# CV-Project2025/Project-NeRF

Measured on AMD Instinct MI355X. Metric: train rays/sec + 800x800 render FPS, NeRF-Synthetic Lego; PSNR parity, higher is better.
Workload: dtype bf16; 1 GPU; Part 2 vanilla NeRF train step (L10/L4 Fourier, 8x256 skip-4 MLP, view 128), batch sampling included; rays_per_gpu=4096, samples_per_ray=64, global_rays=4096, parallelism=ray-dp1, weights=random init (seed 0), frames=100 x 800x800 RGBA resident in HBM (uniform noise)

## Files before the change

include/nerf_hip.h:

```cpp
#ifndef NERF_HIP_H
#define NERF_HIP_H

#include <stddef.h>
#include <stdint.h>

#ifdef __cplusplus
extern "C" {
#endif

#define NERF_OK 0
#define NERF_EINVAL (-22)
#define NERF_ELAUNCH (-5)
#define NERF_ENOSYS (-38)

#define NERF_ABI_VERSION 11

typedef void* nerf_stream_t;

const char* nerf_last_error(void);
int nerf_abi_version(void);

int nerf_set_option(const char* name, int value);
int nerf_get_option(const char* name, int* value_out);

int nerf_sample_rays(const float* rays_o, const float* rays_d, const float* u,
                     int64_t n_rays, int n_samples, float near_plane, float far_plane,
                     float* z_out, float* pts_out, float* dirs_out, nerf_stream_t stream);

int nerf_gather_rays(const float* images, const float* poses, const int64_t* img_idx, const int64_t* pix_y,
                     const int64_t* pix_x, int64_t batch, int n_images, int H, int W, float focal,
                     float scene_scale, float* rays_o, float* rays_d, float* rgba, nerf_stream_t stream);

int nerf_gather_batch(const float* images, const float* poses, const int64_t* flat_idx, int64_t batch, int n_images,
                      int H, int W, float focal, float scene_scale, const float* bg, float* rays_o, float* rays_d,
                      float* rgba, float* target, nerf_stream_t stream);

int nerf_train_batch(const float* images, const float* poses, int n_images, int H, int W, float focal,
                     float scene_scale, const float* bg, uint64_t seed, uint64_t counter, int64_t batch,
                     int n_samples, float near_plane, float far_plane, int perturb, float* rays_o, float* rays_d,
                     float* rgba, float* target, float* z_out, nerf_stream_t stream);

int nerf_train_batch_shard(const float* images, const float* poses, int n_images, int H, int W, float focal,
                     float scene_scale, const float* bg, uint64_t seed, uint64_t counter, int64_t first_ray, int64_t batch,
                     int n_samples, float near_plane, float far_plane, int perturb, float* rays_o, float* rays_d,
                     float* rgba, float* target, float* z_out, nerf_stream_t stream);

int nerf_active_mask(const float* pts, int64_t n, const uint8_t* binary_grid, int resolution,
                     float bound, uint8_t* mask_out, int64_t* idx_out, nerf_stream_t stream);

int nerf_sample_compact(const float* rays_o, const float* rays_d, const float* u, int64_t n_rays,
                        int n_samples, float near_plane, float far_plane, const uint8_t* binary_grid,
                        int resolution, float bound, float* z_out, int* slot_of_sample, float* pts_compact,
                        float* dirs_compact, unsigned* active_count, nerf_stream_t stream);
int nerf_sample_compact_jitter(const float* rays_o, const float* rays_d, uint64_t seed, uint64_t counter,
                               int64_t n_rays, int n_samples, float near_plane, float far_plane,
                               const uint8_t* binary_grid, int resolution, float bound, float* z_out,
                               int* slot_of_sample, float* pts_compact, float* dirs_compact,
                               unsigned* active_count, nerf_stream_t stream);
int nerf_sample_compact_jitter_shard(const float* rays_o, const float* rays_d, uint64_t seed, uint64_t counter,
                                     int64_t first_ray, int64_t n_rays, int n_samples, float near_plane, float far_plane,
                                     const uint8_t* binary_grid, int resolution, float bound, float* z_out,
                                     int* slot_of_sample, float* pts_compact, float* dirs_compact,
                                     unsigned* active_count, nerf_stream_t stream);
#define NERF_COMPACT_CHAIN_WORDS 40
int nerf_sample_compact_jitter_chain(const float* rays_o, const float* rays_d, uint64_t seed, uint64_t counter,
                                     int64_t first_ray, int64_t n_rays, int n_samples, float near_plane, float far_plane,
                                     const uint8_t* binary_grid, int resolution, float bound, float* z_out,
                                     int* slot_of_sample, float* pts_compact, float* dirs_compact,
                                     unsigned* chain_state, int turn, unsigned* count_host, unsigned seq, nerf_stream_t stream);

int nerf_train_batch_compact(const float* images, const float* poses, int n_images, int H, int W, float focal,
                             float scene_scale, const float* bg, uint64_t seed, uint64_t counter, int64_t first_ray,
                             int64_t batch, int n_samples, float near_plane, float far_plane,
                             const uint8_t* binary_grid, int resolution, float bound, float* rays_o, float* rays_d,
                             float* rgba, float* target, float* z_out, int* slot_of_sample, float* pts_compact,
                             float* dirs_compact, unsigned* active_count, nerf_stream_t stream);
int nerf_train_batch_compact_chain(const float* images, const float* poses, int n_images, int H, int W, float focal,
                                   float scene_scale, const float* bg, uint64_t seed, uint64_t counter, int64_t first_ray,
                                   int64_t batch, int n_samples, float near_plane, float far_plane,
                                   const uint8_t* binary_grid, int resolution, float bound, float* rays_o, float* rays_d,
                                   float* rgba, float* target, float* z_out, int* slot_of_sample, float* pts_compact,
                                   float* dirs_compact, unsigned* chain_state, int turn, unsigned* count_host, unsigned seq,
                                   nerf_stream_t stream);

size_t nerf_sample_compact_ordered_scratch_bytes(int64_t n_rays, int n_samples);
int nerf_sample_compact_ordered(const float* rays_o, const float* rays_d, const float* u, int draw, uint64_t seed, uint64_t counter,
                                int64_t first_ray, int64_t n_rays, int n_samples, float near_plane, float far_plane,
                                const uint8_t* binary_grid, int resolution, float bound, float* z_out, int* slot_of_sample,
                                float* pts_compact, float* dirs_compact, unsigned* active_count, void* scratch,
                                size_t scratch_bytes, nerf_stream_t stream);

int nerf_sample_pdf(const float* z_coarse, const float* weights, const float* u, int64_t n_rays,
                    int n_coarse, int n_fine, float* z_out, nerf_stream_t stream);

int nerf_grid_lattice(float bound, int resolution, float* pts_out, nerf_stream_t stream);
int nerf_grid_update(const float* sigma, float* grid, uint8_t* binary_grid, int64_t n_cells,
                     float decay, int dynamic, float threshold, unsigned long long* active_count,
                     nerf_stream_t stream);

int nerf_fourier_encode(const float* x, int64_t n, int dim, int n_freq, float* out,
                        nerf_stream_t stream);

int nerf_composite_fwd(const float* rgb, const float* sigma, const float* z, const float* rays_d,
                       const float* bg, int64_t bg_rows, const float* extra,
                       int64_t n_rays, int n_samples,
                       float* out_rgb, float* out_depth, float* out_acc,
                       float* extra_map, float* weights_out, nerf_stream_t stream);

int nerf_composite_bwd(const float* rgb, const float* sigma, const float* z, const float* rays_d,
                       const float* bg, int64_t bg_rows, const float* extra,
                       const float* g_rgb, const float* g_depth, const float* g_acc,
                       const float* g_extra, int64_t n_rays, int n_samples,
                       float* d_rgb, float* d_sigma, float* d_extra, nerf_stream_t stream);

int nerf_composite_fwd_indexed(const float* rgb_compact, const float* sigma_compact, const int* slot_of_sample,
                               const float* z, const float* rays_d, const float* bg, int64_t bg_rows,
                               int64_t n_rays, int n_samples, float* out_rgb, float* out_depth,
                               float* out_acc, nerf_stream_t stream);
int nerf_composite_bwd_indexed(const float* rgb_compact, const float* sigma_compact, const int* slot_of_sample,
                               const float* z, const float* rays_d, const float* bg, int64_t bg_rows,
                               const float* g_rgb, const float* g_depth, const float* g_acc, int64_t n_rays,
                               int n_samples, float* d_rgb_compact, float* d_sigma_compact,
                               nerf_stream_t stream);

#define NERF_MLP_PARAM_COUNT 595844

size_t nerf_mlp_packed_bytes(void);
int nerf_mlp_pack(const float* params_f32, void* packed, nerf_stream_t stream);
int nerf_mlp_pack_streams(const float* params_f32, void* packed, int which, nerf_stream_t stream);

size_t nerf_mlp_stash_bytes(int64_t n);
int nerf_mlp_fwd(const void* packed, const float* rays_o, const float* rays_d, const float* z,
                 int64_t n, int n_samples, float* rgb, float* sigma, void* stash,
                 nerf_stream_t stream);

int nerf_mlp_fwd_encoded(const void* packed, const float* x_enc, const float* d_enc, int64_t n, float* rgb,
                         float* sigma, void* stash, nerf_stream_t stream);

size_t nerf_mlp_bwd_workspace_bytes(int64_t n);
int nerf_mlp_bwd(const void* packed, const void* stash, const float* rgb, const float* sigma,
                 const float* d_rgb, const float* d_sigma, int64_t n, float* grads_f32,
                 void* workspace, nerf_stream_t stream);
int nerf_mlp_bwd_dgrad(const void* packed, const void* stash, const float* rgb, const float* sigma,
                       const float* d_rgb, const float* d_sigma, int64_t n, void* workspace,
                       nerf_stream_t stream);
int nerf_mlp_bwd_dgrad_ex(const void* packed, const void* stash, const float* rgb, const float* sigma,
// ... 254 lines not shown
```

project-nerf_amd/_lib.py:

```python
import ctypes
import os

_HERE = os.path.dirname(os.path.abspath(__file__))
LIB_PATH = os.path.join(_HERE, "libnerf_hip.so")

c_f32p = ctypes.c_void_p
c_ptr = ctypes.c_void_p
i64 = ctypes.c_int64
i32 = ctypes.c_int
f32 = ctypes.c_float
size_t = ctypes.c_size_t

PROTOTYPES = {
    "nerf_last_error": (ctypes.c_char_p, []),
    "nerf_abi_version": (i32, []),
    "nerf_set_option": (i32, [ctypes.c_char_p, i32]),
    "nerf_get_option": (i32, [ctypes.c_char_p, ctypes.POINTER(i32)]),
    "nerf_sample_rays": (i32, [c_ptr, c_ptr, c_ptr, i64, i32, f32, f32, c_ptr, c_ptr, c_ptr, c_ptr]),
    "nerf_gather_rays": (i32, [c_ptr, c_ptr, c_ptr, c_ptr, c_ptr, i64, i32, i32, i32, f32, f32, c_ptr, c_ptr, c_ptr, c_ptr]),
    "nerf_gather_batch": (i32, [c_ptr, c_ptr, c_ptr, i64, i32, i32, i32, f32, f32, c_ptr, c_ptr, c_ptr, c_ptr, c_ptr, c_ptr]),
    "nerf_train_batch": (i32, [c_ptr, c_ptr, i32, i32, i32, f32, f32, c_ptr, ctypes.c_uint64, ctypes.c_uint64, i64, i32, f32, f32,
                               i32, c_ptr, c_ptr, c_ptr, c_ptr, c_ptr, c_ptr]),
    "nerf_train_batch_shard": (i32, [c_ptr, c_ptr, i32, i32, i32, f32, f32, c_ptr, ctypes.c_uint64, ctypes.c_uint64, i64, i64, i32, f32, f32,
                                     i32, c_ptr, c_ptr, c_ptr, c_ptr, c_ptr, c_ptr]),
    "nerf_active_mask": (i32, [c_ptr, i64, c_ptr, i32, f32, c_ptr, c_ptr, c_ptr]),
    "nerf_sample_compact": (i32, [c_ptr, c_ptr, c_ptr, i64, i32, f32, f32, c_ptr, i32, f32, c_ptr, c_ptr, c_ptr, c_ptr, c_ptr, c_ptr]),
    "nerf_sample_compact_jitter": (i32, [c_ptr, c_ptr, ctypes.c_uint64, ctypes.c_uint64, i64, i32, f32, f32, c_ptr, i32, f32,
                                         c_ptr, c_ptr, c_ptr, c_ptr, c_ptr, c_ptr]),
    "nerf_sample_compact_jitter_shard": (i32, [c_ptr, c_ptr, ctypes.c_uint64, ctypes.c_uint64, i64, i64, i32, f32, f32, c_ptr, i32, f32,
                                               c_ptr, c_ptr, c_ptr, c_ptr, c_ptr, c_ptr]),
    "nerf_sample_compact_jitter_chain": (i32, [c_ptr, c_ptr, ctypes.c_uint64, ctypes.c_uint64, i64, i64, i32, f32, f32, c_ptr, i32, f32,
                                               c_ptr, c_ptr, c_ptr, c_ptr, c_ptr, i32, c_ptr, ctypes.c_uint32, c_ptr]),
    "nerf_train_batch_compact": (i32, [c_ptr, c_ptr, i32, i32, i32, f32, f32, c_ptr, ctypes.c_uint64, ctypes.c_uint64, i64, i64, i32, f32, f32,
                                       c_ptr, i32, f32, c_ptr, c_ptr, c_ptr, c_ptr, c_ptr, c_ptr, c_ptr, c_ptr, c_ptr, c_ptr]),
    "nerf_train_batch_compact_chain": (i32, [c_ptr, c_ptr, i32, i32, i32, f32, f32, c_ptr, ctypes.c_uint64, ctypes.c_uint64, i64, i64, i32, f32,
                                             f32, c_ptr, i32, f32, c_ptr, c_ptr, c_ptr, c_ptr, c_ptr, c_ptr, c_ptr, c_ptr, c_ptr, i32, c_ptr,
                                             ctypes.c_uint32, c_ptr]),
    "nerf_composite_fwd_indexed": (i32, [c_ptr, c_ptr, c_ptr, c_ptr, c_ptr, c_ptr, i64, i64, i32, c_ptr, c_ptr, c_ptr, c_ptr]),
    "nerf_composite_bwd_indexed": (i32, [c_ptr, c_ptr, c_ptr, c_ptr, c_ptr, c_ptr, i64, c_ptr, c_ptr, c_ptr, i64, i32, c_ptr, c_ptr, c_ptr]),
    "nerf_sample_pdf": (i32, [c_ptr, c_ptr, c_ptr, i64, i32, i32, c_ptr, c_ptr]),
    "nerf_grid_lattice": (i32, [f32, i32, c_ptr, c_ptr]),
    "nerf_grid_update": (i32, [c_ptr, c_ptr, c_ptr, i64, f32, i32, f32, c_ptr, c_ptr]),
    "nerf_fourier_encode": (i32, [c_ptr, i64, i32, i32, c_ptr, c_ptr]),
    "nerf_composite_fwd": (i32, [c_ptr, c_ptr, c_ptr, c_ptr, c_ptr, i64, c_ptr, i64, i32,
                                 c_ptr, c_ptr, c_ptr, c_ptr, c_ptr, c_ptr]),
    "nerf_composite_bwd": (i32, [c_ptr, c_ptr, c_ptr, c_ptr, c_ptr, i64, c_ptr, c_ptr, c_ptr, c_ptr,
                                 c_ptr, i64, i32, c_ptr, c_ptr, c_ptr, c_ptr]),
    "nerf_render_rays_workspace_bytes": (size_t, [i64, i32]),
    "nerf_render_rays_fwd": (i32, [c_ptr, c_ptr, c_ptr, i64, i32, f32, f32, c_ptr, i64, i64, c_ptr, c_ptr, c_ptr, c_ptr, c_ptr]),
    "nerf_instant_render_workspace_bytes": (size_t, [i64, i32]),
    "nerf_instant_render_rays_fwd": (i32, [c_ptr, c_ptr, c_ptr, i32, c_ptr, c_ptr, c_ptr, c_ptr, c_ptr, f32, c_ptr, i32, f32, c_ptr, c_ptr, i64, i32,
                                           f32, f32, c_ptr, i64, i64, c_ptr, c_ptr, c_ptr, c_ptr, c_ptr]),
    "nerf_render_rays_grid_workspace_bytes": (size_t, [i64, i32]),
    "nerf_render_rays_grid_fwd": (i32, [c_ptr, c_ptr, i32, f32, c_ptr, c_ptr, i64, i32, f32, f32, c_ptr, i64, i64, c_ptr, c_ptr, c_ptr, c_ptr,
                                        c_ptr]),
    "nerf_mlp_packed_bytes": (size_t, []),
    "nerf_mlp_pack": (i32, [c_ptr, c_ptr, c_ptr]),
    "nerf_mlp_pack_streams": (i32, [c_ptr, c_ptr, i32, c_ptr]),
    "nerf_mlp_stash_bytes": (size_t, [i64]),
    "nerf_mlp_fwd": (i32, [c_ptr, c_ptr, c_ptr, c_ptr, i64, i32, c_ptr, c_ptr, c_ptr, c_ptr]),
    "nerf_mlp_fwd_encoded": (i32, [c_ptr, c_ptr, c_ptr, i64, c_ptr, c_ptr, c_ptr, c_ptr]),
    "nerf_mlp_bwd_workspace_bytes": (size_t, [i64]),
    "nerf_mlp_bwd": (i32, [c_ptr, c_ptr, c_ptr, c_ptr, c_ptr, c_ptr, i64, c_ptr, c_ptr, c_ptr]),
    "nerf_mlp_bwd_dgrad": (i32, [c_ptr, c_ptr, c_ptr, c_ptr, c_ptr, c_ptr, i64, c_ptr, c_ptr]),
    "nerf_mlp_bwd_wgrad": (i32, [c_ptr, c_ptr, i64, c_ptr, c_ptr]),
    "nerf_mlp_bwd_dgrad_ex": (i32, [c_ptr, c_ptr, c_ptr, c_ptr, c_ptr, c_ptr, i64, c_ptr, c_ptr, c_ptr]),
    "nerf_composite_mse_bwd": (i32, [c_ptr, c_ptr, c_ptr, c_ptr, c_ptr, c_ptr, i64, c_ptr, f32, i64, i32, c_ptr, c_ptr,
                                     c_ptr, c_ptr, c_ptr, c_ptr, c_ptr]),
    "nerf_mlp_wgrad_part_split": (i64, []),
    "nerf_mlp_bwd_wgrad_part": (i32, [c_ptr, c_ptr, i64, c_ptr, i32, c_ptr]),
    "nerf_hash_encode_fwd": (i32, [c_ptr, i64, c_ptr, i32, c_ptr, c_ptr, c_ptr, c_ptr, c_ptr, f32, c_ptr, c_ptr, c_ptr, c_ptr]),
    "nerf_hash_encode_fwd_f16": (i32, [c_ptr, i64, c_ptr, i32, c_ptr, c_ptr, c_ptr, c_ptr, c_ptr, f32, c_ptr, c_ptr, c_ptr]),
    "nerf_hash_encode_fwd_nat": (i32, [c_ptr, i64, c_ptr, c_ptr, i32, c_ptr, c_ptr, c_ptr, c_ptr, c_ptr, f32, c_ptr, i32, c_ptr]),
    "nerf_hash_encode_fwd_nat_tables": (i32, [c_ptr, i64, c_ptr, i32, i64, i32, c_ptr, c_ptr, c_ptr, c_ptr, c_ptr, f32, c_ptr, i64, i32, c_ptr]),
    "nerf_f32_to_f16": (i32, [c_ptr, c_ptr, i64, c_ptr]),
    "nerf_hash_encode_bwd": (i32, [c_ptr, i64, i32, c_ptr, c_ptr, c_ptr, c_ptr, c_ptr, f32, c_ptr, c_ptr, c_ptr]),
    "nerf_hash_encode_bwd_levels": (i32, [c_ptr, i64, i32, c_ptr, c_ptr, c_ptr, c_ptr, c_ptr, f32, c_ptr, c_ptr, i32, i32, c_ptr]),
    "nerf_hash_encode_bwd_workspace_bytes": (size_t, [i64, i32]),
    "nerf_hash_encode_bwd_ws": (i32, [c_ptr, i64, i32, c_ptr, c_ptr, c_ptr, c_ptr, c_ptr, f32, c_ptr, c_ptr, i32, i32, c_ptr, size_t, c_ptr]),
    "nerf_hash_encode_bwd_ws_store": (i32, [c_ptr, i64, i32, c_ptr, c_ptr, c_ptr, c_ptr, c_ptr, f32, c_ptr, c_ptr, i32, i32, c_ptr, size_t, c_ptr]),
    "nerf_hash_encode_bwd_tables_workspace_bytes": (size_t, [i64, i32, i32]),
    "nerf_hash_encode_bwd_ws_store_tables": (i32, [c_ptr, i64, i32, i64, i32, c_ptr, c_ptr, c_ptr, c_ptr, c_ptr, f32, c_ptr, i64, c_ptr, c_ptr, size_t, c_ptr]),
    "nerf_hash_encode_bwd_ws_store_tables_spec": (i32, [c_ptr, i64, i32, i64, i32, c_ptr, c_ptr, c_ptr, c_ptr, c_ptr, f32, c_ptr, i64, c_ptr, c_ptr, size_t,
                                                        c_ptr, c_ptr]),
    "nerf_hash_encode_fwd_f16_hist": (i32, [c_ptr, i64, c_ptr, i32, c_ptr, c_ptr, c_ptr, c_ptr, c_ptr, f32, c_ptr, c_ptr, size_t, c_ptr]),
    "nerf_hash_encode_bwd_ws_slots": (i32, [c_ptr, i64, i32, ctypes.POINTER(c_ptr), ctypes.POINTER(c_ptr)]),
    "nerf_hash_encode_bwd_ws_store_precounted": (i32, [c_ptr, i64, i32, c_ptr, c_ptr, c_ptr, c_ptr, c_ptr, f32, c_ptr, c_ptr, size_t, c_ptr]),
    "nerf_hash_encode_bwd_spec_begin": (i32, [c_ptr, c_ptr]),
    "nerf_hash_encode_bwd_ws_store_spec": (i32, [c_ptr, i64, i32, c_ptr, c_ptr, c_ptr, c_ptr, c_ptr, f32, c_ptr, c_ptr, c_ptr, size_t, c_ptr, c_ptr]),
    "nerf_imlp_bwd_amax": (i32, [c_ptr, c_ptr, c_ptr, c_ptr, c_ptr, c_ptr, i64, c_ptr, c_ptr, c_ptr, c_ptr]),
    "nerf_hash_encode_bwd_spec_status": (c_ptr, [c_ptr]),
    "nerf_imlp_bwd_lm": (i32, [c_ptr, c_ptr, c_ptr, c_ptr, c_ptr, c_ptr, i64, c_ptr, c_ptr, c_ptr, c_ptr]),
    "nerf_hash_encode_bwd_input": (i32, [c_ptr, i64, c_ptr, i32, c_ptr, c_ptr, c_ptr, c_ptr, c_ptr, f32, c_ptr, c_ptr, c_ptr]),
# ... 21 lines not shown
    "nerf_p4_workspace_bytes": (size_t, [i64]),
    "nerf_p4_infer_workspace_bytes": (size_t, [i64]),
    "nerf_p4_workspace_offset": (size_t, [i64, i32]),
    "nerf_p4_pack": (i32, [c_ptr, c_ptr, c_ptr]),
    "nerf_p4_sample_inputs": (i32, [c_ptr, c_ptr, c_ptr, i64, i32, f32, f32, ctypes.c_uint64, ctypes.c_uint64, i64, c_ptr, c_ptr, c_ptr]),
    "nerf_p4_deform_fwd": (i32, [c_ptr, c_ptr, c_ptr, c_ptr, c_ptr, c_ptr, i64, c_ptr, c_ptr, i32, c_ptr]),
    "nerf_p4_canon_fwd": (i32, [c_ptr, c_ptr, c_ptr, c_ptr, i64, c_ptr, c_ptr, i32, c_ptr]),
    "nerf_p4_canon_bwd": (i32, [c_ptr, c_ptr, c_ptr, c_ptr, c_ptr, c_ptr, i64, c_ptr, c_ptr, c_ptr, c_ptr]),
    "nerf_p4_deform_bwd": (i32, [c_ptr, c_ptr, c_ptr, c_ptr, i64, c_ptr, c_ptr, c_ptr, c_ptr]),
    "nerf_p3_deform_param_count": (i64, []),
    "nerf_p3_deform_packed_bytes": (size_t, []),
    "nerf_p3_deform_workspace_bytes": (size_t, [i64]),
    "nerf_p3_deform_pack": (i32, [c_ptr, c_ptr, c_ptr]),
    "nerf_p3_deform_fwd": (i32, [c_ptr, c_ptr, c_ptr, c_ptr, c_ptr, i64, c_ptr, c_ptr, i32, c_ptr]),
    "nerf_p3_deform_bwd": (i32, [c_ptr, c_ptr, c_ptr, i64, c_ptr, c_ptr]),
    "nerf_p3_canon_param_count": (i64, [i32]),
    "nerf_p3_canon_packed_bytes": (size_t, []),
    "nerf_p3_canon_workspace_bytes": (size_t, [i64]),
    "nerf_p3_canon_pack": (i32, [c_ptr, i32, c_ptr, c_ptr]),
    "nerf_p3_canon_fwd": (i32, [c_ptr, c_ptr, c_ptr, c_ptr, c_ptr, i64, c_ptr, c_ptr, i32, c_ptr]),
    "nerf_p3_canon_bwd": (i32, [c_ptr, c_ptr, c_ptr, c_ptr, c_ptr, c_ptr, c_ptr, i64, i32, c_ptr, c_ptr, c_ptr]),
    "nerf_p1_param_count": (i64, [i32, i32, i32, i32]),
    "nerf_p1_packed_bytes": (size_t, [i32, i32, i32, i32]),
    "nerf_p1_workspace_bytes": (size_t, [i64, i32, i32, i32, i32]),
    "nerf_p1_pack": (i32, [c_ptr, i32, i32, i32, i32, c_ptr, c_ptr]),
    "nerf_p1_fwd": (i32, [c_ptr, c_ptr, i64, i32, i32, i32, i32, c_ptr, c_ptr]),
    "nerf_p1_fwd_loss_bwd": (i32, [c_ptr, c_ptr, c_ptr, c_ptr, c_ptr, i64, i32, i32, i32, i32, c_ptr, c_ptr, c_ptr]),
    "nerf_p2_param_count": (i64, [i32] * 6),
    "nerf_p2_packed_bytes": (size_t, [i32] * 6),
    "nerf_p2_workspace_bytes": (size_t, [i64] + [i32] * 6),
    "nerf_p2_pack": (i32, [c_ptr] + [i32] * 6 + [c_ptr, c_ptr]),
    "nerf_p2_fwd": (i32, [c_ptr, c_ptr, c_ptr, c_ptr, i64, i32] + [i32] * 6 + [c_ptr, c_ptr, c_ptr]),
    "nerf_p2_fwd_train": (i32, [c_ptr, c_ptr, c_ptr, c_ptr, c_ptr, i64, i32] + [i32] * 6 + [c_ptr, c_ptr, c_ptr]),
    "nerf_p2_bwd": (i32, [c_ptr, c_ptr, c_ptr, c_ptr, c_ptr, c_ptr, i64] + [i32] * 6 + [c_ptr, c_ptr]),
    "nerf_imlp_shape_param_count": (i64, [i32] * 3),
    "nerf_imlp_shape_packed_bytes": (size_t, [i32] * 3),
    "nerf_imlp_shape_workspace_bytes": (size_t, [i64] + [i32] * 3),
    "nerf_imlp_shape_hash_operand_offset": (size_t, [i64] + [i32] * 3),
    "nerf_imlp_shape_pack": (i32, [c_ptr] + [i32] * 3 + [c_ptr, c_ptr]),
    "nerf_imlp_shape_fwd": (i32, [c_ptr, c_ptr, c_ptr, i64] + [i32] * 3 + [c_ptr, c_ptr, i32, c_ptr]),
    "nerf_imlp_shape_bwd": (i32, [c_ptr, c_ptr, c_ptr, c_ptr, c_ptr, c_ptr, i64] + [i32] * 3 + [c_ptr, c_ptr, c_ptr]),
    "nerf_tv_codes_bytes": (size_t, [i64]),
    "nerf_tv_normsq_codes": (i32, [c_ptr, c_ptr, i64, i32, f32, f32, c_ptr, i32, c_ptr, c_ptr]),
    "nerf_clip_adamw_small": (i32, [c_ptr, c_ptr, c_ptr, c_ptr, i64, i32, f32, f32, f32, f32, f32, f32, f32, c_ptr, i32, c_ptr]),
    "nerf_adamw_clip_step_tv": (i32, [c_ptr, c_ptr, c_ptr, c_ptr, i64, i32, f32, f32, f32, f32, f32, c_ptr, f32, f32, c_ptr, i64, f32, i64,
                                      f32, i64, i64, f32, c_ptr, c_ptr]),
    "nerf_tv_normsq_codes_piece": (i32, [c_ptr, c_ptr, i64, i64, i32, f32, f32, c_ptr, i32, c_ptr, c_ptr]),
    "nerf_adamw_clip_step_tv_piece": (i32, [c_ptr, c_ptr, c_ptr, c_ptr, i64, i32, f32, f32, f32, f32, f32, c_ptr, f32, f32, c_ptr, f32, i64, i32,
                                            c_ptr, c_ptr]),
    "nerf_adamw_clip_step": (i32, [c_ptr, c_ptr, c_ptr, c_ptr, i64, i32, f32, f32, f32, f32, f32, c_ptr, f32, f32, c_ptr]),
    "nerf_adamw_clip_step_shadow": (i32, [c_ptr, c_ptr, c_ptr, c_ptr, i64, i32, f32, f32, f32, f32, f32, c_ptr, f32, f32, c_ptr, c_ptr]),
}

ABI_VERSION = 11

_lib = None


class NerfHipError(RuntimeError):
    pass


def load():
    global _lib
    if _lib is not None:
        return _lib
    if not os.path.exists(LIB_PATH):
        raise NerfHipError(
            f"{LIB_PATH} not found: build it with `python project-nerf_amd/build.py` "
            "(hipcc --offload-arch=gfx950).  There is no fallback path.")
    import torch
    lib = ctypes.CDLL(LIB_PATH, mode=ctypes.RTLD_GLOBAL)
    for name, (res, args) in PROTOTYPES.items():
        fn = getattr(lib, name)
        fn.restype = res
        fn.argtypes = args
    if lib.nerf_abi_version() != ABI_VERSION:
        raise NerfHipError(f"ABI version mismatch: {LIB_PATH} reports {lib.nerf_abi_version()}, this binding was written against "
                           f"{ABI_VERSION} (rebuild with `python project-nerf_amd/build.py`)")
    _lib = lib
    return lib


NORMSQ_WS_FLOATS = 4136
COMPACT_CHAIN_WORDS = 40
SUM_WS_FLOATS = 12288


def set_option(name: str, value: int) -> None:
    check(load().nerf_set_option(name.encode(), int(value)), f"nerf_set_option({name})")


def get_option(name: str) -> int:
    out = i32(0)
    check(load().nerf_get_option(name.encode(), ctypes.byref(out)), f"nerf_get_option({name})")
    return out.value


def check(code, what):
    if code != 0:
        msg = load().nerf_last_error().decode("utf-8", "replace")
        raise NerfHipError(f"{what} failed ({code}): {msg}")
```

project-nerf_amd/csrc/hierarchical.hip:

```cpp
#include "common.h"

namespace nerf {

constexpr int kMaxCoarse = 256, kMaxTotal = 1024;

__device__ __forceinline__ float wave_inclusive_sum(float v) {
  v += dpp_row_shr<1>(v, 0.0f);
  v += dpp_row_shr<2>(v, 0.0f);
  v += dpp_row_shr<4>(v, 0.0f);
  v += dpp_row_shr<8>(v, 0.0f);
  const int lane = __lane_id();
  const float r0 = lane_read(v, 15), r1 = lane_read(v, 31), r2 = lane_read(v, 47);
  const int row = lane >> 4;
  return v + (row == 0 ? 0.0f : (row == 1 ? r0 : (row == 2 ? r0 + r1 : r0 + r1 + r2)));
}

__global__ void __launch_bounds__(64)
sample_pdf_kernel(const float* __restrict__ z, const float* __restrict__ weights, const float* __restrict__ u,
                  int64_t R, int S, int NF, int P, float* __restrict__ z_out) {
  __shared__ float cdf[kMaxCoarse];
  __shared__ float bins[kMaxCoarse];
  __shared__ float vals[kMaxTotal];
  const int lane = threadIdx.x;
  const int nb = S - 1;
  const int K = (nb + 63) / 64;
  for (int64_t r = blockIdx.x; r < R; r += gridDim.x) {
    const float* zr = z + r * S;
    const float* wr = weights + r * S;
    float local[4], sum = 0.0f;
    for (int k = 0; k < K; ++k) {
      const int i = lane * K + k;
      local[k] = i < S - 2 ? wr[i + 1] + 1e-5f : 0.0f;
      sum += local[k];
    }
    const float incl = wave_inclusive_sum(sum);
    const float total = lane_read(incl, 63);
    float run = incl - sum;
    for (int k = 0; k < K; ++k) {
      const int i = lane * K + k;
      if (i < nb) {
        cdf[i] = run / total;
        bins[i] = 0.5f * (zr[i + 1] + zr[i]);
      }
      run += local[k];
    }
    __syncthreads();
    const float ustep = NF > 1 ? 1.0f / (float)(NF - 1) : 0.0f;
    for (int j = lane; j < NF; j += 64) {
      float uj;
      if (u != nullptr) uj = u[r * NF + j];
      else uj = (j < NF / 2 || NF == 1) ? ustep * (float)j : __builtin_fmaf(-ustep, (float)(NF - 1 - j), 1.0f);
      int lo = 0, hi = nb;
      while (lo < hi) {
        const int mid = (lo + hi) >> 1;
        if (cdf[mid] <= uj) lo = mid + 1; else hi = mid;
      }
      const int below = lo - 1 > 0 ? lo - 1 : 0, above = lo < nb - 1 ? lo : nb - 1;
      float denom = cdf[above] - cdf[below];
      if (denom < 1e-5f) denom = 1.0f;
      const float t = (uj - cdf[below]) / denom;
      vals[S + j] = bins[below] + t * (bins[above] - bins[below]);
    }
    for (int i = lane; i < S; i += 64) vals[i] = zr[i];
    for (int i = S + NF + lane; i < P; i += 64) vals[i] = __builtin_inff();
    __syncthreads();
    for (int k = 2; k <= P; k <<= 1) {
      for (int j = k >> 1; j > 0; j >>= 1) {
        for (int i = lane; i < P; i += 64) {
          const int l = i ^ j;
          if (l > i) {
            const float a = vals[i], b = vals[l];
            const bool up = (i & k) == 0;
            if ((a > b) == up) { vals[i] = b; vals[l] = a; }
          }
        }
        __syncthreads();
      }
    }
    for (int i = lane; i < S + NF; i += 64) z_out[r * (S + NF) + i] = vals[i];
    __syncthreads();
  }
}

}

extern "C" int nerf_sample_pdf(const float* z_coarse, const float* weights, const float* u, int64_t n_rays,
                               int n_coarse, int n_fine, float* z_out, nerf_stream_t stream) {
  using namespace nerf;
  NERF_REQUIRE(n_rays >= 0 && n_coarse >= 3 && n_coarse <= kMaxCoarse && n_fine >= 1 && n_coarse + n_fine <= kMaxTotal,
               "nerf_sample_pdf: n_coarse=%d (3..%d), n_fine=%d, total <= %d", n_coarse, kMaxCoarse, n_fine, kMaxTotal);
  if (n_rays == 0) return NERF_OK;
  NERF_REQUIRE(z_coarse && weights && z_out, "nerf_sample_pdf: NULL pointer");
  int P = 2;
  while (P < n_coarse + n_fine) P <<= 1;
  int64_t blocks = n_rays < 65536 ? n_rays : 65536;
  hipLaunchKernelGGL(sample_pdf_kernel, dim3((int)blocks), dim3(64), 0, as_stream(stream), z_coarse, weights, u, n_rays,
                     n_coarse, n_fine, P, z_out);
  return check_launch("nerf_sample_pdf");
}
```

project-nerf_amd/engine.py:

```python
from __future__ import annotations

import os
from typing import Dict, Optional, Tuple

import torch

from . import flat_params, ops
from .flat_engine import LapSlots, ViewSlots, cosine_lr, render_chunks

Tensor = torch.Tensor


def param_shapes():
    return [(k, shape) for k, _, shape in flat_params.nerf_decoder_table("", 63, 27)]


def default_init(seed: int = 0) -> Tensor:
    g = torch.Generator().manual_seed(seed)
    parts, fan_in = [], 1
    for name, shape in param_shapes():
        if name.endswith("weight"):
            fan_in = shape[1]
        parts.append(((torch.rand(shape, generator=g) * 2 - 1) / fan_in ** 0.5).reshape(-1))
    return torch.cat(parts)
# ... 8 lines not shown


class VanillaNerfEngine:
    def __init__(self, params: Optional[Tensor] = None, device: str = "cuda", lr: float = 5e-4,
                 near: float = 2.0, far: float = 6.0, white_bkgd: bool = True, seed: int = 0,
                 world_size: int = 1, grid_resolution: int = 128, bound: float = 1.5, grid_threshold: float = 0.01):
        self.device = torch.device(device)
        flat = default_init(seed) if params is None else params.detach().float().reshape(-1)
        assert flat.numel() == ops.MLP_PARAM_COUNT
        self.params = flat.to(self.device).contiguous()
        self.exp_avg = torch.zeros_like(self.params)
        self.exp_avg_sq = torch.zeros_like(self.params)
        self.grads = torch.empty_like(self.params)
        self.packed = torch.empty(ops.mlp_packed_bytes(), dtype=torch.uint8, device=self.device)
        self.lr, self.near, self.far = lr, near, far
        self.bg = (torch.ones(3) if white_bkgd else torch.zeros(3)).to(self.device)
        self.step_count = 0
        self.world_size = world_size
        self.grad_scale = torch.full((1,), 1.0 / world_size, device=self.device)
        self._ws: Dict[Tuple[str, int], Tensor] = {}
        self._scalars = torch.zeros(2, 1024, device=self.device)
        self._slots = LapSlots(self._scalars)
        self._infer_stale = False
        self.grid_resolution, self.bound, self.grid_threshold = int(grid_resolution), float(bound), float(grid_threshold)
        self.grid: Optional[Tensor] = None
        self.binary_grid: Optional[Tensor] = None
        self._grid_ws: Dict[Tuple[int, int], Tensor] = {}
        self.seed, self._jitter_counter = int(seed), 0
        self._grid_train_ws: Dict[str, Tensor] = {}
        self.repack()

    def repack(self, training_only: bool = False) -> None:
        ops.mlp_pack(self.params, self.packed, which=1 if training_only else 3)
        self._infer_stale = training_only

    def _inference_weights(self) -> Tensor:
        if self._infer_stale:
            ops.mlp_pack(self.params, self.packed, which=2)
            self._infer_stale = False
        return self.packed

    def state_dict(self, prefix: str = "decoder.") -> Dict[str, Tensor]:
        return {k: v.clone() for k, v in unflatten(self.params, prefix).items()}

    def load_state_dict(self, sd: Dict[str, Tensor], prefix: str = "decoder.") -> None:
        self.params.copy_(flatten_state_dict(sd, prefix).to(self.device))
        self.repack()

    def _buf(self, kind: str, nbytes: int) -> Tensor:
        key = (kind, nbytes)
        if key not in self._ws:
            self._ws[key] = torch.empty(nbytes, dtype=torch.uint8, device=self.device)
        return self._ws[key]

    GRID_SLACK = (1.25, 1 << 20)

    def _grid_buf(self, kind: str, nbytes: int) -> Tensor:
        buf = self._grid_train_ws.get(kind)
        if buf is None or buf.numel() < nbytes:
            buf = None
            self._grid_train_ws.pop(kind, None)
            buf = self._grid_train_ws[kind] = torch.empty(int(nbytes * self.GRID_SLACK[0]) + self.GRID_SLACK[1], dtype=torch.uint8,
                                                          device=self.device)
        return buf

    def prepare_batch(self, rays_o: Tensor, rays_d: Tensor, n_samples: int = 64, u: Optional[Tensor] = None, first_ray: int = 0):
        grid = self._require_grid("prepare_batch")
        jitter = None
        if u is None:
            self._jitter_counter += 1
            jitter = (self.seed, self._jitter_counter)
        return ops.sample_compact_async(rays_o, rays_d, self.near, self.far, n_samples, grid, self.bound, u=u, jitter=jitter,
                                        first_ray=first_ray)

    def _grid_gradients(self, rays_o: Tensor, rays_d: Tensor, target: Tensor, n_samples: int, u, sync_grads, sync_grads_async, mark,
                        prepared) -> Tensor:
        mark = mark or (lambda name: None)
        if prepared is None:
            prepared = self.prepare_batch(rays_o, rays_d, n_samples, u=u)
        z, slots, pts, dirs = prepared.get()
        mark("sample")
        R, n = rays_o.shape[0], pts.shape[0]
        if n == 0:
            self.grads.zero_()
            loss = ((self.bg.expand(R, 3) - target) ** 2).mean()
            mark("fwd")
            mark("loss")
            mark("dgrad")
            if sync_grads_async is not None:
                split = ops._lib.load().nerf_mlp_wgrad_part_split()
                for h in [sync_grads_async(view) for view in (self.grads[split:], self.grads[:split])]:
                    if h is not None:
                        h.wait()
            mark("wgrad")
            if sync_grads is not None:
                sync_grads(self.grads)
            return loss
        stash = self._grid_buf("stash", ops.mlp_stash_bytes(n))
        rgb, sigma = ops.mlp_fwd(self.packed, pts, dirs, None, stash)
        mark("fwd")
        loss, amax = self._slots.take()
        d_rgb, d_sigma, _ = ops.composite_mse_bwd(rgb, sigma, z, rays_d, self.bg, target, loss, slots=slots, amax_accum=amax)
        mark("loss")
        ws = self._grid_buf("bwd", ops.mlp_bwd_workspace_bytes(n))
        if sync_grads_async is not None:
            ops.mlp_bwd_overlapped(self.packed, stash, rgb, sigma, d_rgb, d_sigma, self.grads, ws, sync_grads_async, amax=amax, mark=mark)
# ... 16 lines not shown
        n = R * n_samples
        if z is None:
            if u is None:
                u = torch.rand(R, n_samples, device=self.device)
            z = ops.sample_rays(rays_o, rays_d, self.near, self.far, n_samples, u=u)
            mark("sample")
        stash = self._buf("stash", ops.mlp_stash_bytes(n))
        rgb, sigma = ops.mlp_fwd(self.packed, rays_o, rays_d, z, stash)
        mark("fwd")
        loss, amax = self._slots.take()
        d_rgb, d_sigma, _ = ops.composite_mse_bwd(rgb.view(R, n_samples, 3), sigma.view(R, n_samples), z, rays_d, self.bg,
                                                  target, loss, amax_accum=amax)
        mark("loss")
        if sync_grads_async is not None:
            ops.mlp_bwd_overlapped(self.packed, stash, rgb, sigma, d_rgb.view(n, 3), d_sigma.view(n), self.grads,
                                   self._buf("bwd", ops.mlp_bwd_workspace_bytes(n)), sync_grads_async, amax=amax, mark=mark)
        else:
            ops.mlp_bwd(self.packed, stash, rgb, sigma, d_rgb.view(n, 3), d_sigma.view(n), self.grads,
                        self._buf("bwd", ops.mlp_bwd_workspace_bytes(n)), amax=amax, mark=mark)
        mark("wgrad")
        if sync_grads is not None:
            sync_grads(self.grads)
        return LapSlots.keep(loss)

    def apply_gradients(self) -> None:
        self.step_count += 1
        ops.adam_step(self.params, self.grads, self.exp_avg, self.exp_avg_sq, self.step_count, self.lr,
                      grad_scale=self.grad_scale if self.world_size > 1 else None)
        self.repack(training_only=True)

    def train_step(self, rays_o: Tensor, rays_d: Tensor, target: Tensor, n_samples: int = 64,
                   u: Optional[Tensor] = None, sync_grads=None, sync_grads_async=None, mark=None,
                   z: Optional[Tensor] = None, grid: bool = False, prepared=None) -> Tensor:
        loss = self.compute_gradients(rays_o, rays_d, target, n_samples, u=u, sync_grads=sync_grads,
                                      sync_grads_async=sync_grads_async, mark=mark, z=z, grid=grid, prepared=prepared)
        self.apply_gradients()
        if mark is not None:
            mark("adam+pack")
        return loss

    @torch.no_grad()
    def render_rays(self, rays_o: Tensor, rays_d: Tensor, n_samples: int, u: Optional[Tensor] = None):
        z = ops.sample_rays(rays_o, rays_d, self.near, self.far, n_samples, u=u)
        rgb, sigma = ops.mlp_fwd(self._inference_weights(), rays_o, rays_d, z)
        R = rays_o.shape[0]
        c, depth, acc, _, _ = ops.composite_fwd(rgb.view(R, n_samples, 3), sigma.view(R, n_samples), z, rays_d, self.bg)
        return c, depth, acc

    @torch.no_grad()
    def render_rays_hierarchical(self, rays_o: Tensor, rays_d: Tensor, n_coarse: int, n_fine: int):
        R = rays_o.shape[0]
        z = ops.sample_rays(rays_o, rays_d, self.near, self.far, n_coarse)
        rgb, sigma = ops.mlp_fwd(self._inference_weights(), rays_o, rays_d, z)
        w = ops.composite_fwd(rgb.view(R, n_coarse, 3), sigma.view(R, n_coarse), z, rays_d, self.bg, want_weights=True)[4]
        z_all = ops.sample_pdf(z, w, n_fine)
        S = n_coarse + n_fine
        rgb, sigma = ops.mlp_fwd(self._inference_weights(), rays_o, rays_d, z_all)
        c, depth, acc, _, _ = ops.composite_fwd(rgb.view(R, S, 3), sigma.view(R, S), z_all, rays_d, self.bg)
        return c, depth, acc

    @torch.no_grad()
    def update_grid(self) -> float:
        res = self.grid_resolution
        pts = ops.grid_lattice(self.bound, res, self.device)
        sig = torch.empty(res ** 3, device=self.device)
        zeros = torch.zeros(2 ** 18, 3, device=self.device)
        packed = self._inference_weights()
        for i in range(0, pts.shape[0], 2 ** 18):
            p = pts[i:i + 2 ** 18]
            sig[i:i + 2 ** 18] = ops.mlp_fwd(packed, p, zeros[:p.shape[0]], None)[1]
        binary, ratio = ops.grid_threshold(sig.view(res, res, res), self.grid_threshold)
        if ratio <= 0.0:
            return 0.0
        self.grid, self.binary_grid = sig.view(res, res, res), binary
        return ratio

    def _require_grid(self, what: str) -> Tensor:
        if self.binary_grid is None:
            raise ValueError(f"{what}: no occupancy grid (call update_grid() or set binary_grid first)")
        return self.binary_grid

    @torch.no_grad()
    def render_rays_grid(self, rays_o: Tensor, rays_d: Tensor, n_samples: int):
        grid = self._require_grid("render_rays_grid")
        z, slots, pts, dirs = ops.sample_compact(rays_o, rays_d, self.near, self.far, n_samples, grid, self.bound)
        R = rays_o.shape[0]
        if pts.shape[0] == 0:
            bg = self.bg.expand(R, 3).clone() if self.bg.dim() == 1 else self.bg.clone()
            return bg, torch.zeros(R, device=self.device), torch.zeros(R, device=self.device)
        rgb, sigma = ops.mlp_fwd(self._inference_weights(), pts, dirs, None)
        return ops.composite_indexed(rgb, sigma, slots, z, rays_d, self.bg)

    def _render_image_grid_chain(self, rays_o: Tensor, rays_d: Tensor, n_samples: int, chunk: int) -> Tensor:
        grid = self._require_grid("render_image(grid=True)")
        shape = rays_o.shape[:-1]
        o, d = rays_o.reshape(-1, 3).contiguous(), rays_d.reshape(-1, 3).contiguous()
        chunk = max(1, min(int(chunk), max(o.shape[0], 1)))
        ws = self._grid_ws.get((chunk, n_samples))
        if ws is None:
            ws = self._grid_ws[(chunk, n_samples)] = torch.empty(ops.render_rays_grid_workspace_bytes(chunk, n_samples), dtype=torch.uint8,
                                                                 device=self.device)
        rgb = ops.render_rays_grid_fwd(self._inference_weights(), grid, self.bound, o, d, n_samples, self.near, self.far, self.bg, chunk,
                                       workspace=ws)[0]
        return rgb.view(*shape, 3)

    @torch.no_grad()
    def render_image(self, rays_o: Tensor, rays_d: Tensor, n_samples: int, chunk: int = 65536, n_fine: int = 0, grid=False) -> Tensor:
        if grid:
            if grid is not True and grid != "loop":
                raise ValueError(f"render_image: grid={grid!r} (False, True or 'loop')")
            if n_fine > 0:
# ... 326 lines not shown
```

project-nerf_amd/ops.py:

```python
from __future__ import annotations

from typing import Optional, Tuple

import torch

from . import _lib

Tensor = torch.Tensor


def _stream() -> int:
    return torch._C._cuda_getCurrentRawStream(torch._C._cuda_getDevice())


def _dev(t: Tensor, name: str, dtype=torch.float32) -> Tensor:
    if not isinstance(t, Tensor):
        raise TypeError(f"{name}: expected a tensor")
    if t.device.type != "cuda":
        raise _lib.NerfHipError(f"{name} is on {t.device}; the hot path only runs on a HIP device (no CPU fallback)")
    if t.dtype != dtype:
        raise TypeError(f"{name}: expected {dtype}, got {t.dtype}")
    return t if t.is_contiguous() else t.contiguous()


# ... 267 lines not shown
                                                  _p(rgba), _p(target), _p(z), _p(slots), _p(pts), _p(dirs), _p(chain.state), turn,
                                                  chain.host[slot].data_ptr(), seq, _stream()), "nerf_train_batch_compact_chain")
    import weakref
    out = CompactedSamples(z, slots, pts, dirs, chain.host_np[slot], None, seq=seq)
    chain.owner[slot] = weakref.ref(out)
    return o, d, (target if bg is not None else rgba), out


class _CompositeIndexed(torch.autograd.Function):
    @staticmethod
    def forward(ctx, rgb_c, sigma_c, slots, z, rays_d, bg):
        lib = _lib.load()
        R, S = z.shape
        rgb_c, sigma_c = _dev(rgb_c, "rgb_c"), _dev(sigma_c, "sigma_c")
        out_rgb = torch.empty(R, 3, device=z.device)
        depth = torch.empty(R, device=z.device)
        acc = torch.empty(R, device=z.device)
        bg_rows = _bg_rows(bg)
        _lib.check(lib.nerf_composite_fwd_indexed(_p(rgb_c), _p(sigma_c), _p(slots), _p(z), _p(rays_d), _p(bg), bg_rows,
                                                  R, S, _p(out_rgb), _p(depth), _p(acc), _stream()),
                   "nerf_composite_fwd_indexed")
        ctx.save_for_backward(rgb_c, sigma_c, slots, z, rays_d, bg)
        return out_rgb, depth, acc

    @staticmethod
    def backward(ctx, g_rgb, g_depth, g_acc):
        lib = _lib.load()
        rgb_c, sigma_c, slots, z, rays_d, bg = ctx.saved_tensors
        R, S = z.shape
        d_rgb, d_sigma = torch.empty_like(rgb_c), torch.empty_like(sigma_c)
        bg_rows = _bg_rows(bg)
        _lib.check(lib.nerf_composite_bwd_indexed(_p(rgb_c), _p(sigma_c), _p(slots), _p(z), _p(rays_d), _p(bg), bg_rows,
                                                  _p(g_rgb.contiguous()), _p(g_depth.contiguous()), _p(g_acc.contiguous()),
                                                  R, S, _p(d_rgb), _p(d_sigma), _stream()), "nerf_composite_bwd_indexed")
        return d_rgb, d_sigma, None, None, None, None


def composite_indexed(rgb_c: Tensor, sigma_c: Tensor, slots: Tensor, z: Tensor, rays_d: Tensor,
                      bg: Optional[Tensor] = None):
    return _CompositeIndexed.apply(rgb_c, sigma_c.reshape(-1), slots, z, rays_d, bg)


def sample_pdf(z_coarse: Tensor, weights: Tensor, n_fine: int, u: Optional[Tensor] = None) -> Tensor:
    lib = _lib.load()
    z_coarse, weights = _dev(z_coarse, "z_coarse"), _dev(weights, "weights")
    R, S = z_coarse.shape
    if u is not None:
        u = _dev(u, "u")
    out = torch.empty(R, S + n_fine, device=z_coarse.device)
    _lib.check(lib.nerf_sample_pdf(_p(z_coarse), _p(weights), _p(u), R, S, n_fine, _p(out), _stream()), "nerf_sample_pdf")
    return out


def grid_lattice(bound: float, resolution: int, device) -> Tensor:
    lib = _lib.load()
    pts = torch.empty(resolution ** 3, 3, device=device, dtype=torch.float32)
    if pts.device.type != "cuda":
        raise _lib.NerfHipError("grid_lattice: the hot path only runs on a HIP device")
    _lib.check(lib.nerf_grid_lattice(float(bound), resolution, _p(pts), _stream()), "nerf_grid_lattice")
    return pts


def grid_threshold(sigma_grid: Tensor, threshold: float, prev: Optional[Tensor] = None, decay: float = 1.0):
    lib = _lib.load()
    cur = _dev(sigma_grid, "sigma_grid")
    grid = cur if prev is None else _dev(prev, "prev")
    binary = torch.empty(cur.shape, device=cur.device, dtype=torch.bool)
    count = torch.zeros(1, device=cur.device, dtype=torch.int64)
    _lib.check(lib.nerf_grid_update(_p(cur), _p(grid), _p(binary), cur.numel(), float(decay),
                                    0 if prev is None else 1, float(threshold), _p(count), _stream()),
               "nerf_grid_update")
    return binary, float(count.item()) / cur.numel()


def fourier_encode(x: Tensor, n_freq: int) -> Tensor:
    lib = _lib.load()
    x = _dev(x, "x")
    n, dim = x.shape
    out = torch.empty(n, dim + 2 * dim * n_freq, device=x.device, dtype=torch.float32)
    _lib.check(lib.nerf_fourier_encode(_p(x), n, dim, n_freq, _p(out), _stream()), "nerf_fourier_encode")
    return out


def composite_fwd(rgb: Tensor, sigma: Tensor, z: Tensor, rays_d: Tensor, bg: Optional[Tensor] = None,
                  extra: Optional[Tensor] = None, want_weights: bool = False):
    lib = _lib.load()
    rgb, sigma, z, rays_d = _dev(rgb, "rgb"), _dev(sigma, "sigma"), _dev(z, "z"), _dev(rays_d, "rays_d")
    R, S = z.shape
    bg = None if bg is None else _dev(bg, "bg")
    bg_rows = _bg_rows(bg)
    out_rgb = torch.empty(R, 3, device=z.device, dtype=torch.float32)
    depth = torch.empty(R, device=z.device, dtype=torch.float32)
    acc = torch.empty(R, device=z.device, dtype=torch.float32)
    extra_map = None
    if extra is not None:
        extra = _dev(extra, "extra")
        extra_map = torch.empty(R, 3, device=z.device, dtype=torch.float32)
    w = torch.empty(R, S, device=z.device, dtype=torch.float32) if want_weights else None
    _lib.check(lib.nerf_composite_fwd(_p(rgb), _p(sigma), _p(z), _p(rays_d), _p(bg), bg_rows, _p(extra),
                                      R, S, _p(out_rgb), _p(depth), _p(acc), _p(extra_map), _p(w), _stream()),
               "nerf_composite_fwd")
    return out_rgb, depth, acc, extra_map, w


def composite_bwd(rgb, sigma, z, rays_d, bg, extra, g_rgb, g_depth, g_acc, g_extra):
    lib = _lib.load()
# ... 628 lines not shown
```

Baseline: 3.951 million rays/s.

## Reuse coarse MLP outputs in hierarchical render, evaluating only fine samples

The hierarchical render path used to run the MLP again over all coarse and fine samples after PDF sampling. The PDF sampler now also writes the fine-only depths and a per-slot source index taken from the bitonic sort. The MLP then runs only on the fine samples, and a merge kernel gathers coarse and fine rgb/sigma into sorted order for compositing. This removes the repeated coarse MLP evaluation, at the cost of an extra gather kernel and some int16 shared-memory swaps during the sort. It affects only the render path, not the train step.

```diff
diff --git a/include/nerf_hip.h b/include/nerf_hip.h
--- a/include/nerf_hip.h
+++ b/include/nerf_hip.h
@@ -13,7 +13,7 @@
 #define NERF_ELAUNCH (-5)
 #define NERF_ENOSYS (-38)
 
-#define NERF_ABI_VERSION 11
+#define NERF_ABI_VERSION 12
 
 typedef void* nerf_stream_t;
 
@@ -92,6 +92,11 @@
 
 int nerf_sample_pdf(const float* z_coarse, const float* weights, const float* u, int64_t n_rays,
                     int n_coarse, int n_fine, float* z_out, nerf_stream_t stream);
+int nerf_sample_pdf_split(const float* z_coarse, const float* weights, const float* u, int64_t n_rays,
+                          int n_coarse, int n_fine, float* z_fine, float* z_all, int16_t* src, nerf_stream_t stream);
+int nerf_merge_two_source(const float* rgb_a, const float* sigma_a, int n_a, const float* rgb_b, const float* sigma_b,
+                          int n_b, const int16_t* src, int64_t n_rays, float* rgb_out, float* sigma_out,
+                          nerf_stream_t stream);
 
 int nerf_grid_lattice(float bound, int resolution, float* pts_out, nerf_stream_t stream);
 int nerf_grid_update(const float* sigma, float* grid, uint8_t* binary_grid, int64_t n_cells,
diff --git a/project-nerf_amd/_lib.py b/project-nerf_amd/_lib.py
--- a/project-nerf_amd/_lib.py
+++ b/project-nerf_amd/_lib.py
@@ -39,6 +39,8 @@
     "nerf_composite_fwd_indexed": (i32, [c_ptr, c_ptr, c_ptr, c_ptr, c_ptr, c_ptr, i64, i64, i32, c_ptr, c_ptr, c_ptr, c_ptr]),
     "nerf_composite_bwd_indexed": (i32, [c_ptr, c_ptr, c_ptr, c_ptr, c_ptr, c_ptr, i64, c_ptr, c_ptr, c_ptr, i64, i32, c_ptr, c_ptr, c_ptr]),
     "nerf_sample_pdf": (i32, [c_ptr, c_ptr, c_ptr, i64, i32, i32, c_ptr, c_ptr]),
+    "nerf_sample_pdf_split": (i32, [c_ptr, c_ptr, c_ptr, i64, i32, i32, c_ptr, c_ptr, c_ptr, c_ptr]),
+    "nerf_merge_two_source": (i32, [c_ptr, c_ptr, i32, c_ptr, c_ptr, i32, c_ptr, i64, c_ptr, c_ptr, c_ptr]),
     "nerf_grid_lattice": (i32, [f32, i32, c_ptr, c_ptr]),
     "nerf_grid_update": (i32, [c_ptr, c_ptr, c_ptr, i64, f32, i32, f32, c_ptr, c_ptr]),
     "nerf_fourier_encode": (i32, [c_ptr, i64, i32, i32, c_ptr, c_ptr]),
@@ -166,7 +168,7 @@
     "nerf_adamw_clip_step_shadow": (i32, [c_ptr, c_ptr, c_ptr, c_ptr, i64, i32, f32, f32, f32, f32, f32, c_ptr, f32, f32, c_ptr, c_ptr]),
 }
 
-ABI_VERSION = 11
+ABI_VERSION = 12
 
 _lib = None
 
diff --git a/project-nerf_amd/csrc/hierarchical.hip b/project-nerf_amd/csrc/hierarchical.hip
--- a/project-nerf_amd/csrc/hierarchical.hip
+++ b/project-nerf_amd/csrc/hierarchical.hip
@@ -15,12 +15,15 @@
   return v + (row == 0 ? 0.0f : (row == 1 ? r0 : (row == 2 ? r0 + r1 : r0 + r1 + r2)));
 }
 
+template <bool kSplit>
 __global__ void __launch_bounds__(64)
 sample_pdf_kernel(const float* __restrict__ z, const float* __restrict__ weights, const float* __restrict__ u,
-                  int64_t R, int S, int NF, int P, float* __restrict__ z_out) {
+                  int64_t R, int S, int NF, int P, float* __restrict__ z_out, float* __restrict__ z_fine,
+                  int16_t* __restrict__ src) {
   __shared__ float cdf[kMaxCoarse];
   __shared__ float bins[kMaxCoarse];
   __shared__ float vals[kMaxTotal];
+  __shared__ int16_t origin[kSplit ? kMaxTotal : 1];
   const int lane = threadIdx.x;
   const int nb = S - 1;
   const int K = (nb + 63) / 64;
@@ -59,10 +62,14 @@
       float denom = cdf[above] - cdf[below];
       if (denom < 1e-5f) denom = 1.0f;
       const float t = (uj - cdf[below]) / denom;
-      vals[S + j] = bins[below] + t * (bins[above] - bins[below]);
+      const float v = bins[below] + t * (bins[above] - bins[below]);
+      vals[S + j] = v;
+      if constexpr (kSplit) z_fine[r * NF + j] = v;
     }
     for (int i = lane; i < S; i += 64) vals[i] = zr[i];
     for (int i = S + NF + lane; i < P; i += 64) vals[i] = __builtin_inff();
+    if constexpr (kSplit)
+      for (int i = lane; i < P; i += 64) origin[i] = (int16_t)i;
     __syncthreads();
     for (int k = 2; k <= P; k <<= 1) {
       for (int j = k >> 1; j > 0; j >>= 1) {
@@ -71,30 +78,85 @@
           if (l > i) {
             const float a = vals[i], b = vals[l];
             const bool up = (i & k) == 0;
-            if ((a > b) == up) { vals[i] = b; vals[l] = a; }
+            if ((a > b) == up) {
+              vals[i] = b; vals[l] = a;
+              if constexpr (kSplit) { const int16_t t = origin[i]; origin[i] = origin[l]; origin[l] = t; }
+            }
           }
         }
         __syncthreads();
       }
     }
     for (int i = lane; i < S + NF; i += 64) z_out[r * (S + NF) + i] = vals[i];
+    if constexpr (kSplit)
+      for (int i = lane; i < S + NF; i += 64) src[r * (S + NF) + i] = origin[i];
     __syncthreads();
+  }
+}
+
+__global__ void __launch_bounds__(256)
+merge_two_source_kernel(const float* __restrict__ rgb_a, const float* __restrict__ sigma_a, int Sa,
+                        const float* __restrict__ rgb_b, const float* __restrict__ sigma_b, int Sb,
+                        const int16_t* __restrict__ src, int64_t R, float* __restrict__ rgb_out, float* __restrict__ sigma_out) {
+  const int lane = threadIdx.x & 63;
+  const int64_t wave = (blockIdx.x * (int64_t)blockDim.x + threadIdx.x) >> 6;
+  const int64_t nwave = ((int64_t)gridDim.x * blockDim.x) >> 6;
+  const int S = Sa + Sb;
+  for (int64_t r = wave; r < R; r += nwave) {
+    for (int k = lane; k < S; k += 64) {
+      int i = src[r * S + k];
+      i = i < 0 ? 0 : (i < S ? i : S - 1);
+      const bool a = i < Sa;
+      const int64_t row = a ? r * Sa + i : r * Sb + (i - Sa);
+      const float* p = (a ? rgb_a : rgb_b) + row * 3;
+      float* o = rgb_out + (r * S + k) * 3;
+      o[0] = p[0];
+      o[1] = p[1];
+      o[2] = p[2];
+      sigma_out[r * S + k] = (a ? sigma_a : sigma_b)[row];
+    }
   }
 }
 
 }
 
-extern "C" int nerf_sample_pdf(const float* z_coarse, const float* weights, const float* u, int64_t n_rays,
-                               int n_coarse, int n_fine, float* z_out, nerf_stream_t stream) {
+template <bool kSplit>
+static int sample_pdf_impl(const float* z_coarse, const float* weights, const float* u, int64_t n_rays, int n_coarse, int n_fine,
+                           float* z_out, float* z_fine, int16_t* src, nerf_stream_t stream) {
   using namespace nerf;
   NERF_REQUIRE(n_rays >= 0 && n_coarse >= 3 && n_coarse <= kMaxCoarse && n_fine >= 1 && n_coarse + n_fine <= kMaxTotal,
                "nerf_sample_pdf: n_coarse=%d (3..%d), n_fine=%d, total <= %d", n_coarse, kMaxCoarse, n_fine, kMaxTotal);
   if (n_rays == 0) return NERF_OK;
-  NERF_REQUIRE(z_coarse && weights && z_out, "nerf_sample_pdf: NULL pointer");
+  NERF_REQUIRE(z_coarse && weights && z_out && (!kSplit || (z_fine && src)), "nerf_sample_pdf: NULL pointer");
   int P = 2;
   while (P < n_coarse + n_fine) P <<= 1;
   int64_t blocks = n_rays < 65536 ? n_rays : 65536;
-  hipLaunchKernelGGL(sample_pdf_kernel, dim3((int)blocks), dim3(64), 0, as_stream(stream), z_coarse, weights, u, n_rays,
-                     n_coarse, n_fine, P, z_out);
-  return check_launch("nerf_sample_pdf");
+  hipLaunchKernelGGL(sample_pdf_kernel<kSplit>, dim3((int)blocks), dim3(64), 0, as_stream(stream), z_coarse, weights, u, n_rays,
+                     n_coarse, n_fine, P, z_out, z_fine, src);
+  return check_launch(kSplit ? "nerf_sample_pdf_split" : "nerf_sample_pdf");
 }
+
+extern "C" int nerf_sample_pdf(const float* z_coarse, const float* weights, const float* u, int64_t n_rays,
+                               int n_coarse, int n_fine, float* z_out, nerf_stream_t stream) {
+  return sample_pdf_impl<false>(z_coarse, weights, u, n_rays, n_coarse, n_fine, z_out, nullptr, nullptr, stream);
+}
+
+extern "C" int nerf_sample_pdf_split(const float* z_coarse, const float* weights, const float* u, int64_t n_rays,
+                                     int n_coarse, int n_fine, float* z_fine, float* z_all, int16_t* src, nerf_stream_t stream) {
+  return sample_pdf_impl<true>(z_coarse, weights, u, n_rays, n_coarse, n_fine, z_all, z_fine, src, stream);
+}
+
+extern "C" int nerf_merge_two_source(const float* rgb_a, const float* sigma_a, int n_a, const float* rgb_b, const float* sigma_b,
+                                     int n_b, const int16_t* src, int64_t n_rays, float* rgb_out, float* sigma_out,
+                                     nerf_stream_t stream) {
+  using namespace nerf;
+  NERF_REQUIRE(n_rays >= 0 && n_a >= 1 && n_b >= 1 && n_a + n_b <= kMaxTotal, "nerf_merge_two_source: n_rays=%lld n_a=%d n_b=%d (total <= %d)",
+               (long long)n_rays, n_a, n_b, kMaxTotal);
+  if (n_rays == 0) return NERF_OK;
+  NERF_REQUIRE(rgb_a && sigma_a && rgb_b && sigma_b && src && rgb_out && sigma_out, "nerf_merge_two_source: NULL pointer");
+  int64_t blocks = (n_rays + 3) / 4;
+  if (blocks > 65536) blocks = 65536;
+  hipLaunchKernelGGL(merge_two_source_kernel, dim3((int)blocks), dim3(256), 0, as_stream(stream), rgb_a, sigma_a, n_a, rgb_b, sigma_b,
+                     n_b, src, n_rays, rgb_out, sigma_out);
+  return check_launch("nerf_merge_two_source");
+}
diff --git a/project-nerf_amd/engine.py b/project-nerf_amd/engine.py
--- a/project-nerf_amd/engine.py
+++ b/project-nerf_amd/engine.py
@@ -84,6 +84,12 @@
         if key not in self._ws:
             self._ws[key] = torch.empty(nbytes, dtype=torch.uint8, device=self.device)
         return self._ws[key]
+
+    def _f32(self, kind: str, *shape: int) -> Tensor:
+        n = 1
+        for s in shape:
+            n *= s
+        return self._buf(kind, 4 * n).view(torch.float32).view(*shape)
 
     GRID_SLACK = (1.25, 1 << 20)
 
@@ -206,11 +212,16 @@
         R = rays_o.shape[0]
         z = ops.sample_rays(rays_o, rays_d, self.near, self.far, n_coarse)
         rgb, sigma = ops.mlp_fwd(self._inference_weights(), rays_o, rays_d, z)
-        w = ops.composite_fwd(rgb.view(R, n_coarse, 3), sigma.view(R, n_coarse), z, rays_d, self.bg, want_weights=True)[4]
-        z_all = ops.sample_pdf(z, w, n_fine)
+        rgb, sigma = rgb.view(R, n_coarse, 3), sigma.view(R, n_coarse)
+        w = ops.composite_fwd(rgb, sigma, z, rays_d, self.bg, want_weights=True)[4]
         S = n_coarse + n_fine
-        rgb, sigma = ops.mlp_fwd(self._inference_weights(), rays_o, rays_d, z_all)
-        c, depth, acc, _, _ = ops.composite_fwd(rgb.view(R, S, 3), sigma.view(R, S), z_all, rays_d, self.bg)
+        z_fine, z_all = self._f32("z_fine", R, n_fine), self._f32("z_all", R, S)
+        src = self._buf("src", 2 * R * S).view(torch.int16).view(R, S)
+        ops.sample_pdf_split(z, w, n_fine, out=(z_fine, z_all, src))
+        rgb_f, sigma_f = ops.mlp_fwd(self._inference_weights(), rays_o, rays_d, z_fine)
+        rgb_all, sigma_all = ops.merge_two_source(rgb, sigma, rgb_f.view(R, n_fine, 3), sigma_f.view(R, n_fine), src,
+                                                  out=(self._f32("rgb_all", R, S, 3), self._f32("sigma_all", R, S)))
+        c, depth, acc, _, _ = ops.composite_fwd(rgb_all, sigma_all, z_all, rays_d, self.bg)
         return c, depth, acc
 
     @torch.no_grad()
diff --git a/project-nerf_amd/ops.py b/project-nerf_amd/ops.py
--- a/project-nerf_amd/ops.py
+++ b/project-nerf_amd/ops.py
@@ -343,6 +343,45 @@
     return out
 
 
+def sample_pdf_split(z_coarse: Tensor, weights: Tensor, n_fine: int, u: Optional[Tensor] = None, out=None):
+    lib = _lib.load()
+    z_coarse, weights = _dev(z_coarse, "z_coarse"), _dev(weights, "weights")
+    R, S = z_coarse.shape
+    if u is not None:
+        u = _dev(u, "u")
+    if out is None:
+        out = (torch.empty(R, n_fine, device=z_coarse.device), torch.empty(R, S + n_fine, device=z_coarse.device),
+               torch.empty(R, S + n_fine, device=z_coarse.device, dtype=torch.int16))
+    z_fine, z_all, src = out
+    for t, name, shape, dtype in ((z_fine, "z_fine", (R, n_fine), torch.float32), (z_all, "z_all", (R, S + n_fine), torch.float32),
+                                  (src, "src", (R, S + n_fine), torch.int16)):
+        if _dev(t, name, dtype) is not t or tuple(t.shape) != shape:
+            raise ValueError(f"{name} must be a contiguous {dtype} tensor of shape {shape}")
+    _lib.check(lib.nerf_sample_pdf_split(_p(z_coarse), _p(weights), _p(u), R, S, n_fine, _p(z_fine), _p(z_all), _p(src), _stream()),
+               "nerf_sample_pdf_split")
+    return z_fine, z_all, src
+
+
+def merge_two_source(rgb_a: Tensor, sigma_a: Tensor, rgb_b: Tensor, sigma_b: Tensor, src: Tensor, out=None):
+    lib = _lib.load()
+    rgb_a, sigma_a, rgb_b, sigma_b = _dev(rgb_a, "rgb_a"), _dev(sigma_a, "sigma_a"), _dev(rgb_b, "rgb_b"), _dev(sigma_b, "sigma_b")
+    src = _dev(src, "src", torch.int16)
+    R, S = src.shape
+    Sa, Sb = sigma_a.shape[-1], sigma_b.shape[-1]
+    if Sa + Sb != S or tuple(sigma_a.shape) != (R, Sa) or tuple(sigma_b.shape) != (R, Sb) or tuple(rgb_a.shape) != (R, Sa, 3) or \
+            tuple(rgb_b.shape) != (R, Sb, 3):
+        raise ValueError(f"merge_two_source: sources of {Sa} + {Sb} samples per ray against src {tuple(src.shape)}")
+    if out is None:
+        out = (torch.empty(R, S, 3, device=src.device), torch.empty(R, S, device=src.device))
+    rgb, sigma = out
+    for t, name, shape in ((rgb, "rgb", (R, S, 3)), (sigma, "sigma", (R, S))):
+        if _dev(t, name) is not t or tuple(t.shape) != shape:
+            raise ValueError(f"{name} must be a contiguous float32 tensor of shape {shape}")
+    _lib.check(lib.nerf_merge_two_source(_p(rgb_a), _p(sigma_a), Sa, _p(rgb_b), _p(sigma_b), Sb, _p(src), R, _p(rgb), _p(sigma), _stream()),
+               "nerf_merge_two_source")
+    return rgb, sigma
+
+
 def grid_lattice(bound: float, resolution: int, device) -> Tensor:
     lib = _lib.load()
     pts = torch.empty(resolution ** 3, 3, device=device, dtype=torch.float32)
```

New measurement: 3.941 million rays/s. No clear change (-0.2%).
